# rafaelcgon/2D-GP

Hardware: AMD Instinct MI355X
Metric: posterior grid points/sec (fit+predict), N_train=4096, div-free 2D kernel (higher is better)
Workload: dtype f64 (variance GEMM as exact int8 Ozaki-II); 1 GPU; df kernel, N_train=4096, 256x256 grid per GPU, fit+predict (mean+variance); n_train=4096, grid_per_gpu=256x256, points_total=65536, parallelism=grid-sharded x1, factor local, kstar_ahead=False

## Files before the change

### 2d-gp_amd/csrc/gp2d.hip

```cpp
#include "common.hpp"
#ifndef GP2D_RELEASE
#error "libgp2d.so is built with -DGP2D_RELEASE=1 (python __graft_entry__.py build)"
#endif
#include "assemble.hpp"
#include "gemm_f64.hpp"
#include "factor.hpp"
#include "predict.hpp"
#include "trend.hpp"
#include "fields.hpp"
#include "grad.hpp"
#include "advect.hpp"
#include "postcov.hpp"
#include "predict_host.hpp"
#include "ozaki.hpp"
#include "ozaki_host.hpp"
#include "factor_host.hpp"
#include "cv.hpp"
#include "lml.hpp"
#include "loo.hpp"
#include "lml_host.hpp"
#include "dfact.hpp"
#include "order.hpp"
#include "../../include/gp2d.h"

// ... 1526 lines not shown

size_t gp2d_predict_ozaki_workspace(int64_t n, int64_t chunk) {
  return OzakiWork(n, chunk, ozaki_nmod_for(n), true).total;
}

size_t gp2d_predict_ozaki_workspace_nmod(int64_t n, int64_t chunk, int nmod) {
  if (nmod <= 0 || nmod > ozaki_nmod_for(n)) return 0;
  return std::max(OzakiWork(n, chunk, nmod, true).total, OzakiWork(n, chunk, nmod, false).total);
}

size_t gp2d_predict_ozaki_planes_workspace(int64_t n, int64_t chunk) {
  return OzakiWork(n, chunk, ozaki_nmod_for(n), false).total;
}

struct OzakiChunk {
  int64_t cv, cp, ncols;
  const double* xg;
  dim3 kgrid;
  OzakiChunk(const double* xg0, int64_t m, int64_t c0, int64_t chunk, int64_t ntr_pad, const gp2d_kernel_t* k)
      : cv(std::min<int64_t>(chunk, m - c0)), cp(round_up(cv, IBN)), ncols(2 * cp), xg(xg0 + point_dim(k) * c0),
        kgrid((unsigned)((ntr_pad + OZ_KS_T - 1) / OZ_KS_T), (unsigned)(cp / OZ_KS_P)) {}
};

static int launch_kstar(const OzakiChunk& c, hipStream_t s, const double* xtr, int64_t ntr, int64_t npad,
                        const VecParams& vp, const double* alpha, const OzakiConsts& oc, int8_t* bres, double* pm,
                        uint8_t* flags) {
  const int form = !ozaki_three(2 * npad) ? KS_PLAIN : oc.pb <= 49 ? KS_DIFF_X : KS_DIFF_R;
  const bool off32 = (uint64_t)(2 * npad) * (uint64_t)c.ncols < (1ull << 31);
  auto launch = [&](auto off32_c, auto form_c) {
    ozaki_kstar_kernel<decltype(off32_c)::value, decltype(form_c)::value>
        <<<c.kgrid, 256, 0, s>>>(xtr, ntr, npad, c.xg, c.cv, c.cp, vp, alpha, oc, bres, pm, flags);
  };
  auto pick = [&](auto off32_c) {
    if (form == KS_PLAIN) launch(off32_c, std::integral_constant<int, KS_PLAIN>{});
    else if (form == KS_DIFF_X) launch(off32_c, std::integral_constant<int, KS_DIFF_X>{});
    else launch(off32_c, std::integral_constant<int, KS_DIFF_R>{});
  };
  if (off32) pick(std::true_type{});
  else pick(std::false_type{});
  return check_launch("ozaki_kstar_kernel");
}

static int predict_ozaki_impl(const int8_t* wres, const double* rowscale, int nmod, int kbits, int64_t n,
                              const double* alpha, const double* xtr, int64_t ntr,
                              int64_t ntr_pad, const double* xg, int64_t m, const gp2d_kernel_t* k, int var_mode,
                              double noise, int compute_var, double* mean, double* var,
                              const int64_t* out_order, int64_t chunk, const OzakiWork& lay, void* work,
                              const KstarBuf* pre, const int8_t* pre_base, hipStream_t s) {
  const auto [bres, cres, pm, P, flags, skip] = lay.at(work);
  OzakiConsts oc;
  GP2D_CHECK(make_ozaki_consts(nmod, k, oc, OZ_PW, ozaki_kbits(kbits)));
  const int nm = oc.nmod;
  GP2D_REQUIRE(n < 131072, "ozaki: the int8 GEMM epilogue needs n < 131072 (N_train < 65536)");
  const int64_t nmseg = (ntr_pad + OZ_KS_T - 1) / OZ_KS_T;
  const int64_t npseg = (n + OZ_CRT_ROWS - 1) / OZ_CRT_ROWS;
  const double kss = gp2d_kernel_diag(k);
  const double add = (var_mode == GP2D_VAR_LATENT) ? 0.0 : noise;
  const int clip = (var_mode == GP2D_VAR_CLIPPED);
  const VecParams vp = make_vec_params(k);
  OzakiConsts oc_mean_only = oc;
  oc_mean_only.nmod = 0;
  int64_t ci = 0;
  for (int64_t c0 = 0; c0 < m; c0 += chunk, ++ci) {
    const OzakiChunk c(xg, m, c0, chunk, ntr_pad, k);
    const int64_t cv = c.cv, cp = c.cp, ncols = c.ncols;
    const int8_t* B = pre ? pre_base + pre->planes_at(ci) : bres;
    const uint8_t* F = pre ? reinterpret_cast<const uint8_t*>(pre_base + pre->flags_at(ci)) : flags;
    const size_t bplane = (size_t)ncols * n;
    const bool inline_planes = compute_var && !pre;
    GP2D_CHECK(launch_kstar(c, s, xtr, ntr, ntr_pad, vp, alpha, inline_planes ? oc : oc_mean_only,
                            pre ? nullptr : bres, pm, inline_planes ? flags : nullptr));
    const int nbj = (int)(ncols / IBN), kslabs = (int)(n / IBK);
    const bool use_skip = compute_var && g_oz_skip && kslabs <= (1 << 20);
    int* slist = skip;
    int* scnt = skip + (int64_t)nbj * kslabs;
    if (use_skip) {
      ozaki_slab_list_kernel<<<(unsigned)nbj, 64, 0, s>>>(F, (int)(ntr_pad / OZ_KS_T), nbj, kslabs, slist, scnt);
      GP2D_CHECK(check_launch("ozaki_slab_list_kernel"));
    }
    if (compute_var) {
      const double nv = 2.0 * (double)ntr;
      TimedLaunch timed(s, 2.0 * (double)cv * nv * nv);
      const bool three = ozaki_three(n);
      const OzakiProducts prods(n, cp, three);
      const int zper = (three || n <= kIgemmZBatchMaxN) ? nm : 1;
      for (int l0 = 0; l0 < nm; l0 += zper) {
        const int nz = std::min(zper, nm - l0);
        IgemmZ zb{(int64_t)n * n, (int64_t)bplane, (int64_t)n * ncols, {}};
        for (int u = 0; u < nz; ++u) zb.m[u] = oc.m[l0 + u];
        constexpr int tbn = 256, nst = I_NSTAGE;
        const int8_t* Al = wres + (size_t)l0 * n * n;
        const int8_t* Bl = B + (size_t)l0 * bplane;
        uint8_t* Cl = cres + (size_t)l0 * n * ncols;
        for (int q = 0; q < prods.count; ++q) {
          const dim3 ggrid(prods.gx[q], prods.gy[q], (unsigned)nz);
          igemm_nt_mod_kernel<tbn, nst><<<ggrid, 2 * tbn, 0, s>>>(Al, Bl, Cl, n, kslabs, oc.m[l0], prods.prod[q],
                                                                  use_skip ? slist : nullptr,
                                                                  use_skip ? scnt : nullptr, zb);
          GP2D_CHECK(check_launch("igemm_nt_mod_kernel"));
        }
      }
      timed.stop();
      const dim3 cgrid((unsigned)((ncols + OZ_CRT_BCOLS - 1) / OZ_CRT_BCOLS), (unsigned)npseg);
      ozaki_crt_colsq_kernel<<<cgrid, 256, 0, s>>>(cres, n, ncols, oc, rowscale, P);
      GP2D_CHECK(check_launch("ozaki_crt_colsq_kernel"));
    }
    GP2D_CHECK(launch_finalize({pm, nmseg, P, npseg, ncols, cp, cv, c0, m, kss, add, clip, compute_var, mean, var,
                                out_order}, s));
  }
  return 0;
}

static int predict_ozaki_args(const gp2d_kernel_t* k, int64_t n, int64_t ntr_pad, int64_t chunk, int var_mode,
                              bool ptrs_ok, int64_t m, int nmod, int kbits, const OzakiWork& lay, const void* work,
                              size_t work_bytes) {
  GP2D_CHECK(validate_ozaki_kernel(k));
  GP2D_REQUIRE(n == 2 * ntr_pad && n % IBM == 0, "ozaki: n must equal 2·ntr_pad and be a multiple of 256");
  GP2D_REQUIRE(chunk > 0 && chunk % (IBN / 2) == 0, "ozaki: chunk must be a positive multiple of 128");
  GP2D_REQUIRE(var_mode >= 0 && var_mode <= 2, "predict: bad var_mode");
  GP2D_REQUIRE(ptrs_ok, "ozaki_planes: alpha and the K* planes are required");
  if (m <= 0) return 1;
  GP2D_REQUIRE(nmod > 0 && nmod <= ozaki_nmod_for(n), "ozaki: nmod exceeds the moduli table");
  GP2D_REQUIRE(work != nullptr && work_bytes >= lay.total, "ozaki: workspace too small");
  return valid_bits(0, kbits);
}

int gp2d_predict_ozaki(const int8_t* wres, const double* rowscale, int nmod, int kbits, int64_t n, const double* alpha,
                       const double* xtr,
                       int64_t ntr, int64_t ntr_pad, const double* xg, int64_t m, const gp2d_kernel_t* k,
                       int var_mode, double noise, int compute_var, double* mean, double* var,
                       const int64_t* out_order, int64_t chunk, void* work, size_t work_bytes, void* stream) {
  const OzakiWork lay(n, chunk, nmod, true);
  const int rc = predict_ozaki_args(k, n, ntr_pad, chunk, var_mode, true, m, nmod, kbits, lay, work, work_bytes);
  if (rc != 0) return rc < 0 ? rc : 0;
  return predict_ozaki_impl(wres, rowscale, nmod, kbits, n, alpha, xtr, ntr, ntr_pad, xg, m, k, var_mode, noise,
                            compute_var, mean, var, out_order, chunk, lay, work, nullptr, nullptr, S(stream));
}

int gp2d_ozaki_nmod_apriori(int64_t n, const gp2d_kernel_t* k, double diag_add, int wbits, int kbits) {
  if (validate_ozaki_kernel(k) != 0 || n <= 0 || valid_bits(wbits, kbits) != 0) return -1;
  const int pw = ozaki_wbits(wbits), pb = ozaki_kbits(kbits);
  const double kss = gp2d_kernel_diag(k);
  const double dmin = (1.0 - std::ldexp(1.0, -40)) / std::sqrt(kss + diag_add);
  const int smax = pw - 1 - (int)std::floor(std::log2(dmin));
  OzakiConsts probe;
  if (make_ozaki_consts(1, k, probe, pw, pb) != 0) return -1;
  const double sq = 2.0 * std::sqrt(kss);
  const double b = std::ldexp(sq, smax + probe.sB) + std::ldexp((double)n, pb - 2) + std::ldexp((double)n, pw) +
                   (double)n;
  const double a_id = 1.01 * std::ldexp(1.0, pw + pb - 2);
  return ozaki_nmod_bits(std::log2(std::max(b, a_id)));
}

size_t gp2d_ozaki_kstar_bytes(int64_t n, int64_t m, int64_t chunk, int nmod) {
  if (n <= 0 || m <= 0 || chunk <= 0 || nmod <= 0) return 0;
  return (size_t)((m + chunk - 1) / chunk) * KstarBuf(n, chunk, nmod).stride;
}

int gp2d_ozaki_kstar(const double* xtr, int64_t ntr, int64_t ntr_pad, const double* xg, int64_t m,
                     const gp2d_kernel_t* k, int nmod, int kbits, int64_t chunk, int8_t* bres, size_t bres_bytes,
                     void* stream) {
  GP2D_CHECK(validate_ozaki_kernel(k));
  const int64_t n = 2 * ntr_pad;
  GP2D_REQUIRE(ntr_pad > 0 && n % IBM == 0 && ntr <= ntr_pad, "ozaki_kstar: 2·ntr_pad must be a multiple of 256");
  GP2D_REQUIRE(chunk > 0 && chunk % (IBN / 2) == 0, "ozaki_kstar: chunk must be a positive multiple of 128");
  GP2D_REQUIRE(nmod > 0 && nmod <= OZ_MAXMOD, "ozaki_kstar: bad number of moduli");
  GP2D_CHECK(valid_bits(0, kbits));
  if (m <= 0) return 0;
  GP2D_REQUIRE(bres != nullptr && bres_bytes >= gp2d_ozaki_kstar_bytes(n, m, chunk, nmod),
               "ozaki_kstar: plane buffer too small");
  OzakiConsts oc;
  GP2D_CHECK(make_ozaki_consts(nmod, k, oc, OZ_PW, ozaki_kbits(kbits)));
  const VecParams vp = make_vec_params(k);
  const KstarBuf buf(n, chunk, nmod);
  hipStream_t s = S(stream);
  int64_t ci = 0;
  for (int64_t c0 = 0; c0 < m; c0 += chunk, ++ci) {
    const OzakiChunk c(xg, m, c0, chunk, ntr_pad, k);
    GP2D_CHECK(launch_kstar(c, s, xtr, ntr, ntr_pad, vp, nullptr, oc, bres + buf.planes_at(ci), nullptr,
                            reinterpret_cast<uint8_t*>(bres + buf.flags_at(ci))));
  }
  return 0;
}

int gp2d_predict_ozaki_planes(const int8_t* wres, const double* rowscale, int nmod, int kbits, int64_t n,
                              const double* alpha, const double* xtr, int64_t ntr, int64_t ntr_pad, const double* xg,
                              int64_t m, const gp2d_kernel_t* k, int var_mode, double noise, const int8_t* bres,
// ... 634 lines not shown
```

### 2d-gp_amd/csrc/ozaki.hpp

```cpp
#pragma once
#include <climits>
#include <type_traits>
#include "common.hpp"
#include "assemble.hpp"

namespace gp2d {

constexpr int OZ_MAXMOD = 20;
#ifdef GP2D_OZ_P
#define GP2D_OZ_PW GP2D_OZ_P
#define GP2D_OZ_PB GP2D_OZ_P
#endif
#ifndef GP2D_OZ_PW
#define GP2D_OZ_PW 49
#endif
#ifndef GP2D_OZ_PB
#define GP2D_OZ_PB 45
#endif
constexpr int OZ_PW = GP2D_OZ_PW;
constexpr int OZ_PB = GP2D_OZ_PB;
static_assert(OZ_PW <= 50 && OZ_PB <= 50, "ozaki: the one-part residues need |x| < 2^50");
constexpr int OZ_PW_MAX = 60;
constexpr int OZ_PB_MAX = 50;
constexpr int OZ_SPLIT = 26;
// ... 310 lines not shown
  int c = 0;
  for (int s0 = 0; s0 < kslabs; s0 += 64) {
    const int sl = s0 + lane;
    bool keep = false;
    if (sl < kslabs) {
      const int tb = sl % ntb;
      keep = (f[tb] | f[ntb + tb] | f[2 * ntb + tb] | f[3 * ntb + tb]) != 0;
    }
    const uint64_t bal = __ballot(keep);
    const int below = c + __popcll(bal & ((1ull << lane) - 1ull));
    if (keep) L[below] = sl;
    if (sl < kslabs && (sl & 3) == 0) C[sl >> 2] = below;
    c += __popcll(bal);
  }
  if (lane == 0) C[kslabs >> 2] = c;
}

struct OzModConsts {
  int neg_c;
  int neg_m;
  uint32_t magic;
};
__host__ __device__ inline uint32_t ozaki_acc_bias(int K, int m) {
  return (uint32_t)((((int64_t)K << 14) + m - 1) / m * m);
}
__device__ __forceinline__ OzModConsts ozaki_mod_consts(int m) {
  OzModConsts c;
  c.neg_c = -((1 << 20) - (1 << 20) % m);
  c.neg_m = -m;
  c.magic = (uint32_t)(((1u << 29) + (uint32_t)m - 1) / (uint32_t)m);
  return c;
}
__device__ __forceinline__ uint32_t ozaki_mod_u32(uint32_t v, const OzModConsts& c) {
  int y, r;
  uint32_t q;
  asm("v_mad_i32_i24 %0, %1, %2, %3" : "=v"(y) : "v"(v >> 20), "s"(c.neg_c), "v"(v));
  asm("v_mul_hi_u32_u24 %0, %1, %2" : "=v"(q) : "s"(c.magic), "v"(y << 3));
  asm("v_mad_i32_i24 %0, %1, %2, %3" : "=v"(r) : "v"(q), "s"(c.neg_m), "v"(y));
  return (uint32_t)r;
}

constexpr int IBM = 256, IBN = 256, IBK = 64;
constexpr int I_OP = IBM * IBK;
constexpr int I_STAGE = 2 * I_OP;
constexpr int I_NSTAGE = 4;


typedef int i4v __attribute__((ext_vector_type(4)));
typedef __attribute__((address_space(3))) void* lds_ptr_t;

__device__ __forceinline__ void lds_dma16(__amdgpu_buffer_rsrc_t r, lds_ptr_t dst, int voff, int soff) {
#if defined(__HIP_DEVICE_COMPILE__)
  __builtin_amdgcn_raw_ptr_buffer_load_lds(r, dst, 16, voff, soff, 0, 0);
#endif
}

__device__ __forceinline__ int swz16(int row, int chunk) {
  const int q = (row >> 2) & 3;
  const int g = (0x78 >> (2 * q)) & 3;
  return chunk ^ g;
}

template <int P, bool BARRIER = true, int W>
__device__ __forceinline__ void vmwait_barrier(std::integral_constant<int, W>) {
  static_assert(P * W < 64, "vmcnt field");
  if constexpr (!BARRIER) {
    asm volatile("s_waitcnt lgkmcnt(0)" ::: "memory");
    return;
  }
  asm volatile("s_waitcnt vmcnt(%0)\n\ts_waitcnt lgkmcnt(0)\n\ts_barrier" ::"n"(P * W) : "memory");
}

struct IgemmProd {
  int bi0;
  int a_slab0;
  int a_fold;
  int a_fold_slab0;
  int b_rb0;
  int b_slab0;
  int alias_rb, alias_ks;
  int k_bi0, k_cap;
  int c_col0;
  int add_col0;
  static IgemmProd plain(int K, bool lower) {
    return {0, 0, INT_MAX, 0, 0, 0, INT_MAX, 0, lower ? 0 : -(1 << 20), K, 0, -1};
  }
};
struct IgemmZ {
  int64_t sA, sB, sC;
  int m[OZ_MAXMOD];
};
constexpr int64_t kIgemmZBatchMaxN = 4096;

struct IgemmNoProbe {
  static constexpr bool kDma = true;
  static constexpr bool kBarrier = true;
  static constexpr bool kLdsRead = true;
  static constexpr bool kMfma = true;
  static constexpr bool kKLoop = true;
  __device__ __forceinline__ void tile_start() {}
  __device__ __forceinline__ void ring_filled() {}
  template <int VM>
  __device__ __forceinline__ void before_wait() {}
  __device__ __forceinline__ void after_barrier() {}
  __device__ __forceinline__ void ring_tail() {}
  __device__ __forceinline__ void before_epilogue() {}
  __device__ __forceinline__ void after_store() {}
};

template <int TBN, int NST, class Probe = IgemmNoProbe>
__global__ __launch_bounds__(TBN * 2, (TBN == 256) ? 1 : 2) void igemm_nt_mod_kernel(
    const int8_t* __restrict__ A, const int8_t* __restrict__ B, uint8_t* C, int64_t ldc, int kslabs_i, int modulus,
    const IgemmProd p, const int* __restrict__ slist, const int* __restrict__ scnt, const IgemmZ zb) {
  Probe probe;
  probe.tile_start();
  if (gridDim.z > 1) {
    A += blockIdx.z * zb.sA;
    B += blockIdx.z * zb.sB;
    C += blockIdx.z * zb.sC;
    modulus = zb.m[blockIdx.z];
  }
  static_assert(TBN == 256 || TBN == 128, "tile width");
  static_assert(NST >= 3 && NST <= 5, "ring depth 3..5 (the tail is written out for these)");
  constexpr int NW = TBN / 32;
  constexpr int WC = TBN / 64;
  constexpr int B_OP = TBN * IBK;
  constexpr int STG = I_OP + B_OP;
  constexpr int AP = IBM / NW / 16;
  constexpr int BPW = TBN / NW / 16;
  constexpr int PPW = AP + BPW;
  __shared__ __attribute__((aligned(16))) int8_t smem[NST * STG];
  const int bj = blockIdx.x;
  const int bi = p.bi0 + (int)(gridDim.y - 1 - blockIdx.y);
  const int i0 = bi * IBM, j0 = bj * TBN;
  const int jb = p.b_rb0 + j0 / IBN, jr = j0 % IBN;
  const int ke = min(p.k_cap, (bi - p.k_bi0 + 1) * IBM);
  const bool afold = bi >= p.a_fold;
  const int arb = afold ? bi - p.a_fold : bi, as0 = afold ? p.a_fold_slab0 : p.a_slab0;
  const int tid = threadIdx.x, lane = tid & 63, wid = __builtin_amdgcn_readfirstlane(tid >> 6);
  const int wr = wid / WC, wc = wid % WC;
  const int l16 = lane & 15, lq = lane >> 4;
  const int64_t kslabs = kslabs_i;
  const int8_t* Ap = A + ((int64_t)arb * kslabs + as0) * I_OP;
  const bool alias = jb >= p.alias_rb;
  const int alias_ks = p.alias_ks;
  const int8_t* Bp = B + ((int64_t)jb * kslabs + p.b_slab0) * I_OP + jr * IBK;
  const int8_t* Bq = B + ((int64_t)(alias ? jb - p.alias_rb : 0) * kslabs + alias_ks) * I_OP + jr * IBK;
  int nsl = ke / IBK;
  const int* sl = nullptr;
  if (slist != nullptr) {
    const int* cn = scnt + (int64_t)jb * (kslabs / 4 + 1) + p.b_slab0 / 4;
    const int c0 = cn[0], c = cn[ke / IBM] - c0;
    if (c == 0 || c >= NST - 1) {
      nsl = c;
      sl = slist + (int64_t)jb * kslabs + c0;
    }
  }
  if constexpr (!Probe::kKLoop) nsl = 0;

  const int bias = (int)ozaki_acc_bias(p.k_cap, modulus);
  i4v acc[8][4];
#pragma unroll
  for (int mi = 0; mi < 8; ++mi)
#pragma unroll
    for (int ni = 0; ni < 4; ++ni) acc[mi][ni] = i4v{bias, bias, bias, bias};

  const int drow = lane >> 2, dchunk = lane & 3;
  const __amdgpu_buffer_rsrc_t rA =
// ... 65 lines not shown
  typedef const __attribute__((address_space(4))) int* const_int_ptr;
  const int b_slab0 = p.b_slab0;
  auto slab = [&](int s) -> int { return sl ? ((const_int_ptr)sl)[min(s, nsl - 1)] - b_slab0 : s; };
  if (nsl > 0) {
#pragma unroll
    for (int q = 0; q < NST - 1; ++q) issue(slab(q), q);
    int knext = slab(NST - 1);
    vmwait_barrier<PPW, Probe::kBarrier>(std::integral_constant<int, NST - 2>{});
    i4v bA[4], a0A[4], bB[4], a0B[4], a1[4];
    if constexpr (!Probe::kLdsRead)
      for (int u = 0; u < 4; ++u) bA[u] = a0A[u] = bB[u] = a0B[u] = a1[u] = i4v{lane, u, wid, 1};
    readb(0, bA);
    reada(0, 0, a0A);
    __builtin_amdgcn_sched_barrier(0);
    probe.ring_filled();
    constexpr int LAST = -1;
    auto step = [&](auto dma_c, auto w_c, int s, i4v (&b)[4], i4v (&a0)[4], i4v (&bn)[4], i4v (&a0n)[4]) {
      constexpr bool dma = decltype(dma_c)::value;
      constexpr int w = decltype(w_c)::value;
      const int st = s % NST;
      if constexpr (dma) {
        issue(knext, (s + NST - 1) % NST);
        knext = slab(s + NST);
      }
      reada(st, 1, a1);
      asm volatile("s_waitcnt lgkmcnt(4)" ::: "memory");
      __builtin_amdgcn_sched_barrier(0);
      mfmas(0, a0, b);
      __builtin_amdgcn_sched_barrier(0);
      if constexpr (w != LAST) {
        if constexpr (dma) probe.template before_wait<PPW * w>();
        vmwait_barrier<PPW, Probe::kBarrier>(w_c);
        if constexpr (dma) probe.after_barrier();
        const int st1 = (s + 1) % NST;
        readb(st1, bn);
        reada(st1, 0, a0n);
        asm volatile("s_waitcnt lgkmcnt(8)" ::: "memory");
      } else {
        asm volatile("s_waitcnt lgkmcnt(0)" ::: "memory");
      }
      __builtin_amdgcn_sched_barrier(0);
      mfmas(1, a1, b);
      __builtin_amdgcn_sched_barrier(0);
    };
    using T_ = std::true_type;
    using F_ = std::false_type;
    using W_FULL = std::integral_constant<int, NST - 2>;
    const int m = nsl - (NST - 1);
    int s = 0;
    for (; s + 1 < m; s += 2) {
      step(T_{}, W_FULL{}, s, bA, a0A, bB, a0B);
      step(T_{}, W_FULL{}, s + 1, bB, a0B, bA, a0A);
    }
    if (s < m) {
      step(T_{}, W_FULL{}, s, bA, a0A, bB, a0B);
      ++s;
#pragma unroll
      for (int u = 0; u < 4; ++u) {
        bA[u] = bB[u];
        a0A[u] = a0B[u];
      }
    }
    probe.ring_tail();
    if constexpr (NST == 5) {
      step(F_{}, std::integral_constant<int, 2>{}, s, bA, a0A, bB, a0B);
      step(F_{}, std::integral_constant<int, 1>{}, s + 1, bB, a0B, bA, a0A);
      step(F_{}, std::integral_constant<int, 0>{}, s + 2, bA, a0A, bB, a0B);
      step(F_{}, std::integral_constant<int, LAST>{}, s + 3, bB, a0B, bA, a0A);
    } else if constexpr (NST == 4) {
      step(F_{}, std::integral_constant<int, 1>{}, s, bA, a0A, bB, a0B);
      step(F_{}, std::integral_constant<int, 0>{}, s + 1, bB, a0B, bA, a0A);
      step(F_{}, std::integral_constant<int, LAST>{}, s + 2, bA, a0A, bB, a0B);
    } else {
      step(F_{}, std::integral_constant<int, 0>{}, s, bA, a0A, bB, a0B);
      step(F_{}, std::integral_constant<int, LAST>{}, s + 1, bB, a0B, bA, a0A);
    }
    asm volatile("s_waitcnt lgkmcnt(0)\n\ts_barrier" ::: "memory");
  }
  probe.before_epilogue();
  uint8_t* T = reinterpret_cast<uint8_t*>(smem);
  constexpr int TP = IBM + 16;
  static_assert(TBN * TP <= NST * STG, "epilogue image fits the ring");
  const OzModConsts mc = ozaki_mod_consts(modulus);
  constexpr int NP = (IBM * TBN / 16) / (TBN * 2);
  auto epilogue = [&](auto add_c) {
    constexpr bool add = decltype(add_c)::value;
    if constexpr (add) {
      const uint8_t* Cp = C + (int64_t)(p.add_col0 + j0) * ldc + i0;
      i4v pv[NP];
#pragma unroll
      for (int q = 0; q < NP; ++q) {
        const int id = tid + TBN * 2 * q;
        pv[q] = __builtin_nontemporal_load(reinterpret_cast<const i4v*>(Cp + (int64_t)(id >> 4) * ldc + 16 * (id & 15)));
      }
#pragma unroll
      for (int q = 0; q < NP; ++q) {
        const int id = tid + TBN * 2 * q;
        *reinterpret_cast<i4v*>(T + (id >> 4) * TP + 16 * (id & 15)) = pv[q];
      }
      __syncthreads();
    }
#pragma unroll
    for (int mi = 0; mi < 8; ++mi)
#pragma unroll
      for (int ni = 0; ni < 4; ++ni) {
        const int rloc = wr * 128 + mi * 16 + 4 * lq;
        const int cloc = wc * 64 + ni * 16 + l16;
        uint32_t* t = reinterpret_cast<uint32_t*>(T + cloc * TP + rloc);
        uint32_t prior = 0;
        if constexpr (add) prior = *t;
        uint32_t pk = 0;
#pragma unroll
        for (int u = 0; u < 4; ++u)
          pk |= ozaki_mod_u32((uint32_t)acc[mi][ni][u] + ((prior >> (8 * u)) & 0xffu), mc) << (8 * u);
        *t = pk;
      }
  };
  if (p.add_col0 >= 0) epilogue(std::true_type{});
  else epilogue(std::false_type{});
  __syncthreads();
  uint8_t* Cc = C + (int64_t)(p.c_col0 + j0) * ldc + i0;
#pragma unroll
  for (int q = 0; q < NP; ++q) {
    const int id = tid + TBN * 2 * q;
    const int cloc = id >> 4, ch = id & 15;
    const i4v v = *reinterpret_cast<const i4v*>(T + cloc * TP + 16 * ch);
    __builtin_nontemporal_store(v, reinterpret_cast<i4v*>(Cc + (int64_t)cloc * ldc + 16 * ch));
  }
  probe.after_store();
}

constexpr int OZ_GUARD_RSEG = 256;
__global__ __launch_bounds__(256) void ozaki_guard_colsq_kernel(const double* __restrict__ W, int64_t n, int64_t ldw,
                                                                double* __restrict__ psum, double* __restrict__ pmax) {
  const int64_t c = (int64_t)blockIdx.x * 256 + threadIdx.x, seg = blockIdx.y;
  const int64_t r0 = seg * OZ_GUARD_RSEG, r1 = min<int64_t>(n, r0 + OZ_GUARD_RSEG);
  if (c >= n) return;
  double sq = 0.0, mx = 0.0;
  if (r1 > (int64_t)blockIdx.x * 256) {
#pragma unroll 8
    for (int64_t r = r0; r < r1; ++r) {
      const double w = W[r * ldw + c];
      sq = fma(w, w, sq);
      mx = fmax(mx, fabs(w));
    }
  }
  psum[seg * n + c] = sq;
  pmax[seg * n + c] = mx;
}

__global__ __launch_bounds__(1024) void ozaki_guard_finish_kernel(const double* __restrict__ psum,
                                                                  const double* __restrict__ pmax, int64_t n,
                                                                  int64_t nseg, int64_t ntr, int64_t npad, double delta,
                                                                  double* __restrict__ stats) {
  __shared__ double red[2][16];
  const int tid = threadIdx.x, lane = tid & 63, w = tid >> 6;
  double vmin = INFINITY, wmax = 0.0;
  for (int64_t c = tid; c < n; c += 1024) {
    double sq = 0.0, mx = 0.0;
    for (int64_t g = 0; g < nseg; ++g) {
      sq += psum[g * n + c];
      mx = fmax(mx, pmax[g * n + c]);
    }
    wmax = fmax(wmax, mx);
    const int64_t loc = c < npad ? c : c - npad;
    if (loc < ntr) vmin = fmin(vmin, delta * (1.0 - delta * sq));
  }
  for (int o = 32; o > 0; o >>= 1) {
    vmin = fmin(vmin, __shfl_xor(vmin, o));
    wmax = fmax(wmax, __shfl_xor(wmax, o));
  }
  if (lane == 0) { red[0][w] = vmin; red[1][w] = wmax; }
  __syncthreads();
  if (tid == 0) {
    for (int q = 1; q < 16; ++q) { vmin = fmin(vmin, red[0][q]); wmax = fmax(wmax, red[1][q]); }
    stats[0] = vmin;
    stats[1] = wmax;
  }
}

__global__ __launch_bounds__(1024) void morton_bbox_kernel(const double* __restrict__ P, int64_t n, int dim,
                                                           double* __restrict__ bbox) {
  __shared__ double red[2][3][32];
  const int tid = threadIdx.x, lane = tid & 63, w = tid >> 6;
  double lo[3] = {INFINITY, INFINITY, INFINITY}, hi[3] = {-INFINITY, -INFINITY, -INFINITY};
  for (int64_t i = tid; i < n; i += 1024)
    for (int c = 0; c < dim; ++c) {
      const double v = P[i * dim + c];
      lo[c] = fmin(lo[c], v);
      hi[c] = fmax(hi[c], v);
    }
  for (int c = 0; c < dim; ++c) {
    for (int o = 32; o > 0; o >>= 1) {
      lo[c] = fmin(lo[c], __shfl_xor(lo[c], o));
      hi[c] = fmax(hi[c], __shfl_xor(hi[c], o));
    }
    if (lane == 0) { red[0][c][w] = lo[c]; red[1][c][w] = hi[c]; }
  }
  __syncthreads();
  if (tid < dim) {
    double a = INFINITY, b = -INFINITY;
    for (int q = 0; q < 16; ++q) { a = fmin(a, red[0][tid][q]); b = fmax(b, red[1][tid][q]); }
    bbox[tid] = a;
    bbox[3 + tid] = b;
  }
}

__device__ __forceinline__ uint64_t spread2(uint64_t v) {
  v = (v | (v << 16)) & 0x0000FFFF0000FFFFull;
  v = (v | (v << 8)) & 0x00FF00FF00FF00FFull;
  v = (v | (v << 4)) & 0x0F0F0F0F0F0F0F0Full;
  v = (v | (v << 2)) & 0x3333333333333333ull;
  return (v | (v << 1)) & 0x5555555555555555ull;
}
__device__ __forceinline__ uint64_t spread3(uint64_t v) {
  v &= 0x1FFFFFull;
  v = (v | (v << 32)) & 0x001F00000000FFFFull;
  v = (v | (v << 16)) & 0x001F0000FF0000FFull;
  v = (v | (v << 8)) & 0x100F00F00F00F00Full;
  v = (v | (v << 4)) & 0x10C30C30C30C30C3ull;
  return (v | (v << 2)) & 0x1249249249249249ull;
}

__global__ __launch_bounds__(256) void morton_code_kernel(const double* __restrict__ P, int64_t n, int dim,
                                                          const double* __restrict__ bbox,
                                                          int64_t* __restrict__ code) {
  const int64_t i = (int64_t)blockIdx.x * 256 + threadIdx.x;
  if (i >= n) return;
  uint64_t c = 0;
  for (int k = 0; k < dim; ++k) {
    const double lo = bbox[k], span = fmax(bbox[3 + k] - lo, 1e-300);
    double q = rint((P[i * dim + k] - lo) / span * 2097151.0);
    q = fmin(fmax(q, 0.0), 2097151.0);
    const uint64_t v = (uint64_t)q;
    c |= (dim == 2 ? spread2(v) : spread3(v)) << k;
  }
  code[i] = (int64_t)c;
}

#ifndef GP2D_CRT_RPL
#define GP2D_CRT_RPL 16
#endif
constexpr int OZ_CRT_RPL = GP2D_CRT_RPL;
static_assert(OZ_CRT_RPL == 16 || OZ_CRT_RPL == 8, "CRT rows per lane: 16 or 8");
constexpr int OZ_CRT_ROWS = 64 * OZ_CRT_RPL;
constexpr int OZ_CRT_COLS = 4;
constexpr int OZ_CRT_BCOLS = 4 * OZ_CRT_COLS;

template <int RPL> struct crt_load;
template <> struct crt_load<16> { typedef uint4 type; };
template <> struct crt_load<8> { typedef uint2 type; };

#ifndef GP2D_CRT_OCC
#define GP2D_CRT_OCC 1
#endif
__global__ __launch_bounds__(256, GP2D_CRT_OCC) void ozaki_crt_colsq_kernel(const uint8_t* __restrict__ cres, int64_t n,
                                                              int64_t ncols, OzakiConsts oc,
                                                              const double* __restrict__ rowscale,
                                                              double* __restrict__ P) {
  constexpr int RPL = OZ_CRT_RPL;
  typedef typename crt_load<RPL>::type ld_t;
  const int lane = threadIdx.x & 63;
  const int64_t jw = (int64_t)blockIdx.x * OZ_CRT_BCOLS + (threadIdx.x >> 6) * OZ_CRT_COLS;
  const int64_t seg = blockIdx.y;
  const int64_t i0 = seg * OZ_CRT_ROWS + RPL * lane;
  if (jw >= ncols) return;
  const bool rows_ok = i0 < n;
  double rs[RPL];
#pragma unroll
  for (int c = 0; c < RPL; ++c) rs[c] = rows_ok ? rowscale[i0 + c] : 0.0;
  const int64_t plane = n * ncols;
#pragma unroll 1
  for (int jc = 0; jc < OZ_CRT_COLS; ++jc) {
    const int64_t j = jw + jc;
    if (j >= ncols) break;
    double acc = 0.0;
    if (rows_ok) {
      double H[RPL], T[RPL];
#pragma unroll
      for (int c = 0; c < RPL; ++c) { H[c] = 0.0; T[c] = 0.0; }
      const int nm1 = oc.nmod - 1;
      for (int l0 = 0; l0 < oc.nmod; l0 += 4) {
        ld_t v[4];
#pragma unroll
        for (int u = 0; u < 4; ++u)
          v[u] = *reinterpret_cast<const ld_t*>(cres + (int64_t)min(l0 + u, nm1) * plane + j * n + i0);
#pragma unroll
        for (int u = 0; u < 4; ++u) {
          const uint32_t* w = reinterpret_cast<const uint32_t*>(&v[u]);
          const double h = oc.h[l0 + u], t = oc.t[l0 + u];
#pragma unroll
          for (int c = 0; c < RPL; ++c) {
            const double cl = (double)((w[c >> 2] >> (8 * (c & 3))) & 0xffu);
            H[c] = fma(cl, h, H[c]);
            T[c] = fma(cl, t, T[c]);
          }
        }
      }
#pragma unroll
      for (int c = 0; c < RPL; ++c) {
        const double f = (H[c] - rint(H[c])) + T[c];
        const double vij = f * rs[c];
        acc = fma(vij, vij, acc);
        if (fabs(vij) > oc.vlimit) acc = __builtin_nan("");
      }
    }
#pragma unroll
    for (int o = 32; o > 0; o >>= 1) acc += __shfl_xor(acc, o);
    if (lane == 0) P[seg * ncols + j] = acc;
  }
}

}
```

### 2d-gp_amd/csrc/ozaki_host.hpp

```cpp
#pragma once
#include <algorithm>
#include "ozaki.hpp"

namespace gp2d {

constexpr size_t oz_flag_bytes(int64_t n, int64_t chunk) {
  return (size_t)round_up((round_up(chunk < 1 ? 1 : chunk, IBN) / OZ_KS_P) * (n / 2 / OZ_KS_T), 256);
}
constexpr size_t oz_list_bytes(int64_t n, int64_t chunk) {
  const int64_t nbj = 2 * round_up(chunk < 1 ? 1 : chunk, IBN) / IBN, ks = n / IBK;
  return sizeof(int) * (size_t)(nbj * ks + nbj * (ks / 4 + 1));
}

struct KstarBuf {
  size_t planes, flag_bytes, stride;
  KstarBuf(int64_t n, int64_t chunk, int nmod)
      : planes((size_t)nmod * (size_t)n * (size_t)(2 * round_up(chunk, IBN))), flag_bytes(oz_flag_bytes(n, chunk)),
        stride(planes + flag_bytes) {}
  size_t planes_at(int64_t ci) const { return (size_t)ci * stride; }
  size_t flags_at(int64_t ci) const { return (size_t)ci * stride + planes; }
};

struct OzakiWork {
  size_t bres = 0, cres = 0, pm = 0, P = 0, flags = 0, skip = 0, total = 0;
  constexpr OzakiWork(int64_t n, int64_t chunk, int nmod, bool inline_planes) {
    if (nmod <= 0 || n <= 0) return;
    const size_t ncols = (size_t)(2 * round_up(chunk < 1 ? 1 : chunk, IBN));
    const size_t plane = (size_t)nmod * (size_t)n * ncols;
    const size_t ks_rows = (size_t)(n / 2 / OZ_KS_T + 1);
    const size_t crt_rows = (size_t)(n / OZ_CRT_ROWS + 1);
    cres = bres + (inline_planes ? plane : 0);
    pm = cres + plane;
    P = pm + sizeof(double) * ncols * (inline_planes ? ks_rows : std::max(ks_rows, crt_rows));
    flags = P + sizeof(double) * ncols * crt_rows;
    skip = flags + (inline_planes ? oz_flag_bytes(n, chunk) : 0);
    total = skip + oz_list_bytes(n, chunk);
  }
  struct Ptrs { int8_t* bres; uint8_t* cres; double* pm; double* P; uint8_t* flags; int* skip; };
  Ptrs at(void* work) const {
    char* w = static_cast<char*>(work);
    return {reinterpret_cast<int8_t*>(w + bres), reinterpret_cast<uint8_t*>(w + cres), reinterpret_cast<double*>(w + pm),
            reinterpret_cast<double*>(w + P), reinterpret_cast<uint8_t*>(w + flags), reinterpret_cast<int*>(w + skip)};
  }
};

constexpr int64_t oz_s_npad(int64_t n) { return (n > 0 && n % (2 * IBM) == 0) ? n / 2 : 0; }

struct OzakiProducts {
  int count;
  IgemmProd prod[3];
  unsigned gx[3], gy[3];
  OzakiProducts(int64_t n, int64_t cp, bool three) {
    const int nb = (int)(n / IBM), nbh = (int)(cp / IBN), hs = (int)(n / 2 / IBK);
    if (!three) {
      count = 1;
      prod[0] = IgemmProd::plain((int)n, true);
      prod[0].alias_rb = nbh;
      prod[0].alias_ks = hs;
      gx[0] = 2u * nbh;
      gy[0] = (unsigned)nb;
      return;
    }
    const int nb2 = nb / 2, npad = (int)(n / 2), vcol = (int)cp;
    count = 3;
    prod[0] = {0,   0,      nb2,    hs,          0,    hs,     INT_MAX, 0,       0,    npad, vcol,  -1};
    prod[1] = {0,   0,      INT_MAX, 0,          0,    0,      INT_MAX, 0,       0,    npad, 0,     vcol};
    prod[2] = {nb2, hs,     INT_MAX, 0,          nbh,  hs,     INT_MAX, 0,       nb2,  npad, vcol,  vcol};
    gx[0] = gx[1] = gx[2] = (unsigned)nbh;
    gy[0] = gy[1] = (unsigned)nb;
    gy[2] = (unsigned)nb2;
  }
};

constexpr bool ozaki_work_ok(int64_t n, int64_t chunk, int nmod) {
  for (int inl = 0; inl < 2; ++inl) {
    const OzakiWork w(n, chunk, nmod, inl);
    if (w.bres != 0 || (w.cres > w.bres) != inl || w.pm <= w.cres || w.P <= w.pm || w.flags <= w.P ||
        w.skip < w.flags || (w.skip > w.flags) != inl || w.total <= w.skip || w.pm % 8 || w.P % 8 || w.skip % 4)
      return false;
  }
  return true;
}
static_assert(ozaki_work_ok(256, 128, 12) && ozaki_work_ok(256, 128, 16) && ozaki_work_ok(8192, 8192, 13),
              "OzakiWork: regions out of order, overlapping or misaligned");

}
```

Before: 1.302 million points/s.

## Fold Ozaki three-product accumulation into the CRT column-square kernel

When the K* planes are built inline, the third integer GEMM product now writes its residues into the spare B-plane buffer instead of read-modify-writing the shared C residues. The first two products also stop accumulating into C. The CRT reduction kernel gains a SUM3 variant that adds the residues modulo m while reconstructing, handling both column halves per thread. This removes the epilogue reload of C in two GEMM launches but makes the CRT kernel read three residue streams and do more integer work.

```diff
diff --git a/2d-gp_amd/csrc/gp2d.hip b/2d-gp_amd/csrc/gp2d.hip
--- a/2d-gp_amd/csrc/gp2d.hip
+++ b/2d-gp_amd/csrc/gp2d.hip
@@ -1632,27 +1632,36 @@
       const double nv = 2.0 * (double)ntr;
       TimedLaunch timed(s, 2.0 * (double)cv * nv * nv);
       const bool three = ozaki_three(n);
-      const OzakiProducts prods(n, cp, three);
+      const OzakiProducts prods(n, cp, three, !pre);
       const int zper = (three || n <= kIgemmZBatchMaxN) ? nm : 1;
       for (int l0 = 0; l0 < nm; l0 += zper) {
         const int nz = std::min(zper, nm - l0);
-        IgemmZ zb{(int64_t)n * n, (int64_t)bplane, (int64_t)n * ncols, {}};
-        for (int u = 0; u < nz; ++u) zb.m[u] = oc.m[l0 + u];
         constexpr int tbn = 256, nst = I_NSTAGE;
         const int8_t* Al = wres + (size_t)l0 * n * n;
         const int8_t* Bl = B + (size_t)l0 * bplane;
-        uint8_t* Cl = cres + (size_t)l0 * n * ncols;
         for (int q = 0; q < prods.count; ++q) {
+          const bool in_b = prods.sum_in_crt && q == 2;
+          uint8_t* Cl = in_b ? reinterpret_cast<uint8_t*>(bres) + (size_t)l0 * bplane + prods.p3_off
+                             : cres + (size_t)l0 * n * ncols;
+          IgemmZ zb{(int64_t)n * n, (int64_t)bplane, in_b ? (int64_t)bplane : (int64_t)n * ncols, {}};
+          for (int u = 0; u < nz; ++u) zb.m[u] = oc.m[l0 + u];
           const dim3 ggrid(prods.gx[q], prods.gy[q], (unsigned)nz);
-          igemm_nt_mod_kernel<tbn, nst><<<ggrid, 2 * tbn, 0, s>>>(Al, Bl, Cl, n, kslabs, oc.m[l0], prods.prod[q],
-                                                                  use_skip ? slist : nullptr,
+          igemm_nt_mod_kernel<tbn, nst><<<ggrid, 2 * tbn, 0, s>>>(Al, Bl, Cl, in_b ? n / 2 : n, kslabs, oc.m[l0],
+                                                                  prods.prod[q], use_skip ? slist : nullptr,
                                                                   use_skip ? scnt : nullptr, zb);
           GP2D_CHECK(check_launch("igemm_nt_mod_kernel"));
         }
       }
       timed.stop();
-      const dim3 cgrid((unsigned)((ncols + OZ_CRT_BCOLS - 1) / OZ_CRT_BCOLS), (unsigned)npseg);
-      ozaki_crt_colsq_kernel<<<cgrid, 256, 0, s>>>(cres, n, ncols, oc, rowscale, P);
+      if (prods.sum_in_crt) {
+        const dim3 cgrid((unsigned)((cp + OZ_CRT_BCOLS - 1) / OZ_CRT_BCOLS), (unsigned)npseg);
+        ozaki_crt_colsq_kernel<true><<<cgrid, 256, 0, s>>>(cres, n, ncols, oc, rowscale, P,
+                                                           reinterpret_cast<const uint8_t*>(bres) + prods.p3_off,
+                                                           (int64_t)bplane, prods.p3_blk);
+      } else {
+        const dim3 cgrid((unsigned)((ncols + OZ_CRT_BCOLS - 1) / OZ_CRT_BCOLS), (unsigned)npseg);
+        ozaki_crt_colsq_kernel<false><<<cgrid, 256, 0, s>>>(cres, n, ncols, oc, rowscale, P, nullptr, 0, 0);
+      }
       GP2D_CHECK(check_launch("ozaki_crt_colsq_kernel"));
     }
     GP2D_CHECK(launch_finalize({pm, nmseg, P, npseg, ncols, cp, cv, c0, m, kss, add, clip, compute_var, mean, var,
diff --git a/2d-gp_amd/csrc/ozaki.hpp b/2d-gp_amd/csrc/ozaki.hpp
--- a/2d-gp_amd/csrc/ozaki.hpp
+++ b/2d-gp_amd/csrc/ozaki.hpp
@@ -416,8 +416,10 @@
   int k_bi0, k_cap;
   int c_col0;
   int add_col0;
+  int64_t c_off;
+  int64_t c_blk;
   static IgemmProd plain(int K, bool lower) {
-    return {0, 0, INT_MAX, 0, 0, 0, INT_MAX, 0, lower ? 0 : -(1 << 20), K, 0, -1};
+    return {0, 0, INT_MAX, 0, 0, 0, INT_MAX, 0, lower ? 0 : -(1 << 20), K, 0, -1, 0, 0};
   }
 };
 struct IgemmZ {
@@ -649,11 +651,15 @@
   constexpr int TP = IBM + 16;
   static_assert(TBN * TP <= NST * STG, "epilogue image fits the ring");
   const OzModConsts mc = ozaki_mod_consts(modulus);
+  auto cat = [&](int col) -> uint8_t* {
+    const int64_t blk = p.c_blk > 0 ? p.c_blk : IBN * ldc;
+    return C + p.c_off + (col / IBN) * blk + (col % IBN) * ldc;
+  };
   constexpr int NP = (IBM * TBN / 16) / (TBN * 2);
   auto epilogue = [&](auto add_c) {
     constexpr bool add = decltype(add_c)::value;
     if constexpr (add) {
-      const uint8_t* Cp = C + (int64_t)(p.add_col0 + j0) * ldc + i0;
+      const uint8_t* Cp = cat(p.add_col0 + j0) + i0;
       i4v pv[NP];
 #pragma unroll
       for (int q = 0; q < NP; ++q) {
@@ -686,7 +692,7 @@
   if (p.add_col0 >= 0) epilogue(std::true_type{});
   else epilogue(std::false_type{});
   __syncthreads();
-  uint8_t* Cc = C + (int64_t)(p.c_col0 + j0) * ldc + i0;
+  uint8_t* Cc = cat(p.c_col0 + j0) + i0;
 #pragma unroll
   for (int q = 0; q < NP; ++q) {
     const int id = tid + TBN * 2 * q;
@@ -821,15 +827,34 @@
 #ifndef GP2D_CRT_OCC
 #define GP2D_CRT_OCC 1
 #endif
+__device__ __forceinline__ double crt_value(double H, double T, double rs) {
+  const double f = (H - rint(H)) + T;
+  return f * rs;
+}
+__device__ __forceinline__ double crt_square_in(double vij, double vlimit, double acc) {
+  acc = fma(vij, vij, acc);
+  if (fabs(vij) > vlimit) acc = __builtin_nan("");
+  return acc;
+}
+__device__ __forceinline__ uint32_t residue_sum(uint32_t r1, uint32_t r2, uint32_t m) {
+  const uint32_t s = r1 + r2;
+  return min(s, s - m);
+}
+
+template <bool SUM3>
 __global__ __launch_bounds__(256, GP2D_CRT_OCC) void ozaki_crt_colsq_kernel(const uint8_t* __restrict__ cres, int64_t n,
                                                               int64_t ncols, OzakiConsts oc,
                                                               const double* __restrict__ rowscale,
-                                                              double* __restrict__ P) {
+                                                              double* __restrict__ P,
+                                                              const uint8_t* __restrict__ p3, int64_t p3_stride,
+                                                              int64_t p3_blk) {
   constexpr int RPL = OZ_CRT_RPL;
-  typedef typename crt_load<RPL>::type ld_t;
   const int lane = threadIdx.x & 63;
   const int64_t jw = (int64_t)blockIdx.x * OZ_CRT_BCOLS + (threadIdx.x >> 6) * OZ_CRT_COLS;
   const int64_t seg = blockIdx.y;
+  const int nm1 = oc.nmod - 1;
+  if constexpr (!SUM3) {
+  typedef typename crt_load<RPL>::type ld_t;
   const int64_t i0 = seg * OZ_CRT_ROWS + RPL * lane;
   if (jw >= ncols) return;
   const bool rows_ok = i0 < n;
@@ -846,7 +871,6 @@
       double H[RPL], T[RPL];
 #pragma unroll
       for (int c = 0; c < RPL; ++c) { H[c] = 0.0; T[c] = 0.0; }
-      const int nm1 = oc.nmod - 1;
       for (int l0 = 0; l0 < oc.nmod; l0 += 4) {
         ld_t v[4];
 #pragma unroll
@@ -865,17 +889,93 @@
         }
       }
 #pragma unroll
-      for (int c = 0; c < RPL; ++c) {
-        const double f = (H[c] - rint(H[c])) + T[c];
-        const double vij = f * rs[c];
-        acc = fma(vij, vij, acc);
-        if (fabs(vij) > oc.vlimit) acc = __builtin_nan("");
-      }
+      for (int c = 0; c < RPL; ++c) acc = crt_square_in(crt_value(H[c], T[c], rs[c]), oc.vlimit, acc);
     }
 #pragma unroll
     for (int o = 32; o > 0; o >>= 1) acc += __shfl_xor(acc, o);
     if (lane == 0) P[seg * ncols + j] = acc;
   }
-}
-
-}
+  } else {
+  constexpr int HR = 8, NPASS = RPL / HR;
+  constexpr bool PAIR = NPASS == 2;
+  const int64_t cp = ncols / 2, npad = n / 2;
+  if (jw >= cp) return;
+  const int64_t plane = n * ncols;
+#pragma unroll 1
+  for (int jc = 0; jc < OZ_CRT_COLS; ++jc) {
+    const int64_t j = jw + jc;
+    if (j >= cp) break;
+    double tot[2] = {0.0, 0.0};
+#pragma unroll
+    for (int pass = 0; pass < NPASS; ++pass) {
+      const int64_t i0 = seg * OZ_CRT_ROWS + pass * (64 * HR) + HR * lane;
+      double acc[2] = {0.0, 0.0};
+      if (i0 < n) {
+        const bool vrow = i0 >= npad;
+        double H[2][HR], T[2][HR];
+#pragma unroll
+        for (int c = 0; c < HR; ++c) H[0][c] = H[1][c] = T[0][c] = T[1][c] = 0.0;
+        const uint8_t* c1 = cres + (cp + j) * n + i0;
+        const uint8_t* c2 = cres + j * n + i0;
+        const uint8_t* c3 = p3 + (j >> 8) * p3_blk + (j & 255) * npad + (i0 - npad);
+        for (int l0 = 0; l0 < oc.nmod; l0 += 4) {
+          uint2 v1[4], v2[4], v3[4];
+#pragma unroll
+          for (int u = 0; u < 4; ++u) {
+            const int64_t lu = min(l0 + u, nm1);
+            v1[u] = *reinterpret_cast<const uint2*>(c1 + lu * plane);
+            v2[u] = *reinterpret_cast<const uint2*>(c2 + lu * plane);
+            v3[u] = vrow ? *reinterpret_cast<const uint2*>(c3 + lu * p3_stride) : make_uint2(0u, 0u);
+          }
+#pragma unroll
+          for (int u = 0; u < 4; ++u) {
+            const uint32_t w1[2] = {v1[u].x, v1[u].y}, w2[2] = {v2[u].x, v2[u].y}, w3[2] = {v3[u].x, v3[u].y};
+            const double h = oc.h[l0 + u], t = oc.t[l0 + u];
+            const uint32_t m = (uint32_t)oc.m[min(l0 + u, nm1)];
+#pragma unroll
+            for (int c = 0; c < HR; ++c) {
+              const int sh = 8 * (c & 3);
+              const uint32_t r1 = (w1[c >> 2] >> sh) & 0xffu, r2 = (w2[c >> 2] >> sh) & 0xffu,
+                             r3 = (w3[c >> 2] >> sh) & 0xffu;
+              const double cu = (double)residue_sum(r1, r2, m), cv = (double)residue_sum(r1, r3, m);
+              H[0][c] = fma(cu, h, H[0][c]);
+              T[0][c] = fma(cu, t, T[0][c]);
+              H[1][c] = fma(cv, h, H[1][c]);
+              T[1][c] = fma(cv, t, T[1][c]);
+            }
+          }
+        }
+        double rs[HR];
+#pragma unroll
+        for (int c = 0; c < HR; ++c) rs[c] = rowscale[i0 + c];
+#pragma unroll
+        for (int e = 0; e < 2; ++e) {
+          double v[HR];
+#pragma unroll
+          for (int c = 0; c < HR; ++c) v[c] = crt_value(H[e][c], T[e][c], rs[c]);
+          double a = 0.0;
+#pragma unroll
+          for (int c = 0; c < HR; ++c) a = crt_square_in(v[c], oc.vlimit, a);
+          if constexpr (PAIR) {
+            a = __shfl(a, lane - 1);
+#pragma unroll
+            for (int c = 0; c < HR; ++c) a = crt_square_in(v[c], oc.vlimit, a);
+          }
+          acc[e] = a;
+        }
+      }
+      tot[0] = pass == 0 ? acc[0] : tot[0] + acc[0];
+      tot[1] = pass == 0 ? acc[1] : tot[1] + acc[1];
+    }
+#pragma unroll
+    for (int e = 0; e < 2; ++e) {
+      double a = tot[e];
+#pragma unroll
+      for (int o = 32; o >= (PAIR ? 2 : 1); o >>= 1) a += __shfl_xor(a, o);
+      if (lane == (PAIR ? 1 : 0)) P[seg * ncols + e * cp + j] = a;
+    }
+  }
+  }
+}
+
+}
diff --git a/2d-gp_amd/csrc/ozaki_host.hpp b/2d-gp_amd/csrc/ozaki_host.hpp
--- a/2d-gp_amd/csrc/ozaki_host.hpp
+++ b/2d-gp_amd/csrc/ozaki_host.hpp
@@ -50,7 +50,9 @@
   int count;
   IgemmProd prod[3];
   unsigned gx[3], gy[3];
-  OzakiProducts(int64_t n, int64_t cp, bool three) {
+  bool sum_in_crt = false;
+  int64_t p3_off = 0, p3_blk = 0;
+  OzakiProducts(int64_t n, int64_t cp, bool three, bool spare) {
     const int nb = (int)(n / IBM), nbh = (int)(cp / IBN), hs = (int)(n / 2 / IBK);
     if (!three) {
       count = 1;
@@ -63,9 +65,14 @@
     }
     const int nb2 = nb / 2, npad = (int)(n / 2), vcol = (int)cp;
     count = 3;
-    prod[0] = {0,   0,      nb2,    hs,          0,    hs,     INT_MAX, 0,       0,    npad, vcol,  -1};
-    prod[1] = {0,   0,      INT_MAX, 0,          0,    0,      INT_MAX, 0,       0,    npad, 0,     vcol};
-    prod[2] = {nb2, hs,     INT_MAX, 0,          nbh,  hs,     INT_MAX, 0,       nb2,  npad, vcol,  vcol};
+    sum_in_crt = spare;
+    p3_off = cp * n;
+    p3_blk = (int64_t)IBN * n;
+    const int add = spare ? -1 : vcol;
+    const int64_t o3 = spare ? -(int64_t)npad : 0, b3 = spare ? p3_blk : 0;
+    prod[0] = {0,   0,      nb2,    hs,          0,    hs,     INT_MAX, 0,       0,    npad, vcol,              -1,      0,    0};
+    prod[1] = {0,   0,      INT_MAX, 0,          0,    0,      INT_MAX, 0,       0,    npad, 0,                 add,     0,    0};
+    prod[2] = {nb2, hs,     INT_MAX, 0,          nbh,  hs,     INT_MAX, 0,       nb2,  npad, spare ? 0 : vcol,  add,     o3,   b3};
     gx[0] = gx[1] = gx[2] = (unsigned)nbh;
     gy[0] = gy[1] = (unsigned)nb;
     gy[2] = (unsigned)nb2;
```

After: 1.317 million points/s (median of 6 runs). 1.1% higher.
